# delehef/asgart

Measured on AMD Instinct MI355X. Metric: Mbp/s probe+extend (direct+RC, k=20 g=100), higher is better.
Workload: dtype u64 keys / u32 SA

## Files before the change

### asgart_amd/csrc/pipeline.hip

```cpp
#include "pipeline_dev.hpp"
#include "extend_wave_dev.hpp"
#include "extend_heavy_dev.hpp"
#include "extend_fast_dev.hpp"
#include "extend_k8_dev.hpp"

#include <algorithm>
#include <atomic>
#include <chrono>
#include <functional>
#include <string>
#include <thread>
#include <utility>

namespace asgart {

#ifdef ASGART_PROFILE_EXTEND
#define PROF_DUMP(tag)                                                                          \
    do {                                                                                       \
        fprintf(stderr, "[extend profile %s] stage=%llu batches=%llu | reg_cyc=%llu reg_probes=%llu | build=%llu "\
                "lds_probes=%llu match=%llu apply=%llu retire=%llu segs=%llu sumA=%llu sumCnt=%llu | longest: "   \
                "cyc=%llu g0=%llu lds_probes=%llu reg_probes=%llu sumA=%llu sumCnt=%llu stage=%llu match=%llu\n", \
                tag, h_ctr[16], h_ctr[17], h_ctr[18], h_ctr[19], h_ctr[20], h_ctr[21], h_ctr[22], h_ctr[23],  \
                h_ctr[24], h_ctr[25], h_ctr[26], h_ctr[27], h_ctr[28], h_ctr[29], h_ctr[30] >> 32,            \
                h_ctr[30] & 0xffffffffull, h_ctr[31] >> 32, h_ctr[31] & 0xffffffffull, h_ctr[32], h_ctr[33]); \
// ... 364 lines not shown
                    set_error("more than 2^32 probes in one call");
                    return ASGART_E_CAP;
                }
            }
            lp[(size_t)n_chunks_pass] = (uint32_t)P64;
        }
        Ppass = lp[(size_t)n_chunks_pass];
        P = Ppass * (uint32_t)n_passes;
        cx.last_P = P;
        memset(&cx.stats, 0, sizeof(cx.stats));
        cx.stats.probes_total = P;
        if (fam_out)
            for (int32_t p = 0; p < n_passes; ++p) {
                fams[p]->fam_offsets.assign(1, 0);
                fams[p]->fam_keys.clear();
                fams[p]->sds.clear();
            }
        if (want_csr) {
            status_out->assign(P, 0);
            rowoff_out->assign((size_t)P + 1, 0);
            hits_out->clear();
        }
        if (P == 0 || n_chunks == 0) return 0;
        if (want_csr && (n_shards != 1 || n_passes != 1)) {
            set_error("asgart_probe_hits is one unsharded pass");
            return ASGART_E_ARG;
        }
        own_lo = (uint32_t)((uint64_t)Ppass * (uint64_t)shard / (uint64_t)n_shards);
        own_hi = (uint32_t)((uint64_t)Ppass * (uint64_t)(shard + 1) / (uint64_t)n_shards);
        if (own_lo == own_hi) return 0;
        look_back = (uint64_t)opt.shard_lookback;
        look_ahead = opt.shard_lookahead > 0 ? (uint64_t)opt.shard_lookahead
                                                      : std::max<uint64_t>(65536, (own_hi - own_lo) / 16);
        const int64_t c0 = (int64_t)(std::upper_bound(lp.begin(), lp.end(), own_lo) - lp.begin()) - 1;
        const int64_t c1 = (int64_t)(std::upper_bound(lp.begin(), lp.end(), own_hi - 1u) - lp.begin()) - 1;
        lo_lim = lp[(size_t)c0];
        hi_lim = lp[(size_t)c1 + 1];
        K = hi_lim - lo_lim;
        for (int64_t c = 0; c < n_chunks; ++c) {
            const int64_t cl = c % n_chunks_pass, p = c / n_chunks_pass;
            h_start[c] = chunks[2 * cl];
            h_len[c] = chunks[2 * cl + 1];
            h_pbase[c] = (uint32_t)p * K + (std::min(std::max(lp[(size_t)cl], lo_lim), hi_lim) - lo_lim);
        }
        h_pbase[n_chunks] = (uint32_t)n_passes * K;
        call_sig = 1469598103934665603ull;
        {
            auto mix = [&](uint64_t v) { call_sig = (call_sig ^ v) * 1099511628211ull; };
            mix(k);
            mix(st->max_gap_size);
            mix(st->min_duplication_length);
            mix(st->max_cardinality);
            for (int64_t c = 0; c < 2 * n_chunks_pass; ++c) mix(chunks[c]);
        }
        RC_TRY(w.chunks.reserve(ch_bytes));
        d_start = w.chunks.as<uint64_t>();
        d_len = d_start + n_chunks;
        d_pbase = reinterpret_cast<uint32_t *>(d_len + n_chunks);
        HIP_TRY(hipMemcpyAsync(d_start, h_start, ch_bytes, hipMemcpyHostToDevice, s));
        t_host0 = std::chrono::steady_clock::now();
        nothing_to_do = false;
        return 0;
    }

    void set_window() {
        const uint32_t w_lo = (uint32_t)std::max<uint64_t>(lo_lim, own_lo > look_back ? own_lo - look_back : 0);
        const uint32_t w_hi = (uint32_t)std::min<uint64_t>(hi_lim, (uint64_t)own_hi + look_ahead);
        rp.init_unknown = w_lo != lo_lim ? 1u : 0u;
        rp.ch = ChunkTable{d_start, d_len, d_pbase, (int)n_chunks};
        rp.win_len = w_hi - w_lo;
        rp.win_stride = K;
        rp.g_lo = w_lo - lo_lim;
        rp.g_hi = rp.g_lo + ((uint32_t)n_passes - 1u) * K + rp.win_len;
        rp.own_off_lo = own_lo - w_lo;
        rp.own_off_hi = own_hi - w_lo;
        W = rp.g_hi - rp.g_lo;
        W_probes = (uint32_t)n_passes * rp.win_len;
        rp.k = (int)k;
        rp.step = (int)step;
        rp.G = st->max_gap_size;
        rp.tstar = (uint32_t)((st->max_gap_size + step - 1) / step);
        if (rp.tstar == 0) rp.tstar = 1;
        rp.M = st->min_duplication_length;
        rp.C = st->max_cardinality > 0xFFFFFF00ull ? 0xFFFFFF00u : (uint32_t)st->max_cardinality;
        rp.n_passes = (uint32_t)n_passes;
        rp.pass_chunks = (uint32_t)n_chunks_pass;
        rp.modes = 0;
        rp.blank = 0;
        for (int p = 0; p < 4; ++p) {
            rp.pbits[p] = nullptr;
            if (p >= n_passes) continue;
            const int mode = (sts[p].reverse ? 2 : 0) | (sts[p].complement ? 1 : 0);
            rp.modes |= (uint32_t)mode << (8 * p);
            rp.pbits[p] = opt.posbits ? idx->d_pbits[mode] : nullptr;
            if (rp.pbits[p] && idx->pbits_uses[mode] == 0) rp.blank |= 1u << p;
        }
        cx.last_rp = rp;
        cx.has_last = false;

    }

    int32_t front(bool *ambiguous) {
        const uint32_t n_blk = rp.n_tiles((uint32_t)kScanTile);
        const uint64_t seg_cap = (uint64_t)W_probes / (rp.tstar + 1) + (uint64_t)n_chunks + 64;
        RC_TRY(reserve_probe_workspace(idx, cx, W));
        RC_TRY(w.seg_list.reserve((size_t)seg_cap * 4));
        RC_TRY(w.counters.reserve(CT_COUNT * 8));
        d_ctr = w.counters.as<unsigned long long>();
        HIP_TRY(hipMemsetAsync(d_ctr, 0, CT_COUNT * 8, s));
        ix = idx->template view<SlotT>();
        p_lo = w.p_lo.as<SlotT>() - rp.g_lo;
        p_raw = w.p_raw.as<uint32_t>() - rp.g_lo;
        p_filt = w.p_filt.as<uint32_t>() - rp.g_lo;
        row_off = w.row_off.as<unsigned long long>() - rp.g_lo;
        unsigned long long *scan_desc = w.blk.as<unsigned long long>();
        uint32_t *big_list = w.big_list.as<uint32_t>();
        uint32_t *rank_list = w.rank_list.as<uint32_t>();
        seg_list = w.seg_list.as<uint32_t>();

        if (opt.test_stall_s > 0) stall_kernel<<<1, 64, 0, s>>>((unsigned long long)opt.test_stall_s * 100000000ull);
        HIP_TRY(hipEventRecord(cx.ev[EV_SEARCH], s));
        probe_count_kernel<SlotT, false><<<rp.n_tiles((uint32_t)kProbeBlock), kProbeThreads, 0, s>>>(
            ix, rp, p_lo, p_raw, p_filt, big_list, rank_list, d_ctr);
        HIP_TRY(hipEventRecord(cx.ev[EV_PROBE_COUNT], s));
        collect_pending_kernel<<<std::min<uint32_t>(rp.n_tiles((uint32_t)kCollectTile), 256u * 8u), kCollectBlock, 0, s>>>(
            rp, p_filt, big_list, rank_list, d_ctr);
        big_count_kernel<SlotT, false><<<2048, 256, 0, s>>>(ix, rp, p_lo, p_raw, p_filt, big_list, d_ctr);
        uint32_t *const ranked_top = big_list + W;
        if (ix.sap)
            rank_count_kernel<SlotT, false><<<2048, 256, 0, s>>>(ix, rp, p_lo, p_raw, p_filt, rank_list, big_list, ranked_top,
                                                                 ix.sar ? idx->ranked_fill : 0, d_ctr);
        HIP_TRY(hipEventRecord(cx.ev[EV_SEARCHED], s));
        HIP_TRY(hipMemsetAsync(scan_desc, 0, (size_t)n_blk * 16, s));
        scan_segments_kernel<<<std::min<uint32_t>(n_blk, 256u * 2u), kScanBlock, 0, s>>>(rp, p_filt, scan_desc, n_blk, row_off, seg_list, d_ctr);
        HIP_TRY(hipEventRecord(cx.ev[EV_SCANNED], s));
        HIP_TRY(hipGetLastError());
        HIP_TRY(hipMemcpyAsync(h_ctr, d_ctr, kCtrBytes, hipMemcpyDeviceToHost, s));
        RC_TRY(wd_sync(idx, cx, s, "the probe search and the scans"));
        total_hits = h_ctr[CT_TOTAL_HITS];
        n_seg = h_ctr[CT_SEG];
        if (h_ctr[CT_AMBIG]) {
            *ambiguous = true;
            return 0;
        }
        if (n_seg > seg_cap) {
            set_error("internal: segment list overflow (%llu > %llu)", (unsigned long long)n_seg,
                      (unsigned long long)seg_cap);
            return ASGART_E_CAP;
        }
        RC_TRY(w.hits.reserve((size_t)(total_hits + 64) * sizeof(SlotT)));
        hits = w.hits.as<SlotT>();
        hipStream_t sf = cx.fill_stream;
        HIP_TRY(hipEventRecord(cx.ev[EV_FILL], sf));
        fill_small_kernel<SlotT><<<rp.n_tiles(256u), 256, 0, sf>>>(ix, rp, p_lo, p_raw, p_filt, row_off, hits);
        if (h_ctr[CT_BIG])
            fill_big_kernel<SlotT><<<2048, 256, 0, sf>>>(ix, rp, p_lo, p_raw, p_filt, row_off, hits,
                                                         big_list, d_ctr);
        if constexpr (sizeof(SlotT) == 4) {
            if (h_ctr[CT_RANKED])
                fill_ranked_kernel<SlotT><<<(unsigned)std::min<uint64_t>((h_ctr[CT_RANKED] + 255) / 256, 4096), 256, 0, sf>>>(
                    ix, rp, p_lo, p_raw, p_filt, row_off, hits, ranked_top, d_ctr);
        }
        HIP_TRY(hipEventRecord(cx.ev[EV_HIT_ROWS], sf));
        HIP_TRY(hipGetLastError());

        return 0;
    }

    int32_t csr_out() {
        std::vector<uint32_t> h_filt(P);
        std::vector<SlotT> h_hits((size_t)total_hits);
        RC_TRY(wd_sync(idx, cx, s, "the hit rows"));
        HIP_TRY(hipMemcpyAsync(h_filt.data(), p_filt, (size_t)P * 4, hipMemcpyDeviceToHost, s));
        HIP_TRY(hipMemcpyAsync(rowoff_out->data(), row_off, ((size_t)P + 1) * 8,
                               hipMemcpyDeviceToHost, s));
        if (total_hits)
            HIP_TRY(hipMemcpyAsync(h_hits.data(), hits, (size_t)total_hits * sizeof(SlotT),
                                   hipMemcpyDeviceToHost, s));
        HIP_TRY(hipStreamSynchronize(s));
        for (uint32_t g = 0; g < P; ++g)
            (*status_out)[g] = h_filt[g] == kSkipN ? 1 : (h_filt[g] == kSkipCard ? 2 : 0);
        hits_out->resize((size_t)total_hits);
        for (uint64_t j = 0; j < total_hits; ++j) (*hits_out)[j] = h_hits[j];
        return 0;
    }

    int32_t place() {
        rec_cap = std::max<uint64_t>(1u << 18, w.fam_sds.cap / sizeof(SdRec));
        RC_TRY(w.ovf_list.reserve((size_t)(n_seg + 1) * 4 * kTiers));
        h_recs = nullptr;
        n_hrec = 0;
        const int force_tier = (int)opt.force_tier;
        RC_TRY(w.seg_keys.reserve((size_t)n_seg * 4 * 2));
        RC_TRY(w.seg_vals.reserve((size_t)n_seg * 4 * 2));
        uint32_t *kbuf = w.seg_keys.as<uint32_t>(), *vbuf = w.seg_vals.as<uint32_t>();
        HIP_TRY(hipMemsetAsync(d_ctr + CT_N1, 0, (size_t)(CT_COUNT - CT_N1) * 8, s));
        arms_kernel = rp.C <= (uint64_t)kHitBatch && opt.arms_kernel != 0 && (uint64_t)idx->n < (1ull << 42);
        for (int t = 1; t <= kTiers; ++t) {
            const TierShape &sh = shape(t);
            const bool usable = sh.kernel != TierKernel::none && !(arms_kernel && rp.C > (uint64_t)sh.hits);
            tier_cap[t] = usable ? (uint32_t)((uint64_t)sh.cap() * (uint64_t)(sh.widen ? opt.*sh.widen : 100) / 100u) : 0u;
        }
        tier_cap[kTiers] = 0xFFFFFFFFu;
        if (arms_kernel)
            tier_cap[3] = std::min(std::max(shape(3).cap(), tier_cap[6]), tier_cap[3]);
        else
            tier_cap[6] = (rp.G >= 0xFFF0u || rp.C >= 0xFFF0u) ? 0u : tier_cap[6] * 7 / 5;
        PlaceParams pp;
        pp.long3 = pp.long3_big = pp.dense3 = pp.dense6 = 0;
        pp.stats = opt.debug ? 1u : 0u;
        pp.barren = opt.barren ? 1u : 0u;
        pp.seg_info = nullptr;
        const bool cluster_barren = opt.barren >= 2 && rp.M > (uint64_t)k;
        split_on = opt.split >= (sizeof(SlotT) == 4 ? 1 : 2) && arms_kernel && (opt.split_len == 0 || opt.split_len >= 64);
        if (cluster_barren || split_on) {
            RC_TRY(w.seg_info.reserve((size_t)n_seg * sizeof(uint2)));
            pp.seg_info = w.seg_info.as<uint2>();
        }
        d_split = nullptr;
        if (split_on) {
            RC_TRY(w.split_buf.reserve(kSplitBytes));
            d_split = w.split_buf.as<char>();
            HIP_TRY(hipMemsetAsync(d_split, 0, 64, s));
        }
        pp.k = (uint32_t)k;
        pp.step = (uint32_t)step;
        pp.G = rp.G;
        pp.M = rp.M;
        for (int t = 1; t < kTiers; ++t) pp.cap[t - 1] = tier_cap[t];
        if (arms_kernel) {
            pp.long3 = (uint32_t)opt.long3;
            pp.long3_big = pp.long3 / 4u;
            pp.dense3 = (uint32_t)opt.dense3;
            pp.dense6 = (uint32_t)opt.dense6;
            if (force_tier == 3) {
                pp.long3 = pp.long3_big = 1;
                pp.dense3 = pp.dense6 = 0;
            }
            pp.cap[0] = (uint32_t)std::min<int64_t>(opt.cap1, shape(1).cap());
        }
        {
            int n_resident = 0;
            for (int t = 2; t < kTiers; ++t)
                n_resident += tier_enabled(t) && (shape(t).kernel == TierKernel::fast || shape(t).kernel == TierKernel::k8) ? 1 : 0;
            const bool on = tail_up.mode == 2 || (tail_up.mode == 1 && cx.n_tier_st < n_resident);
            for (int t = 1; t < kTiers; ++t) {
                const bool source = (t == 2 || t == 4 || t == 5) && shape(t).kernel == TierKernel::fast;
                const uint32_t thr = !source ? 0u : tail_up.hits > 0 ? (uint32_t)std::min<int64_t>(tail_up.hits, 0xFFFFFFFFll) : shape(t).tail_hits;
                pp.tail_hits[t - 1] = tail_hits[t] = on && tier_enabled(t) ? thr : 0u;
            }
        }
        int force_eff = force_tier;
        while (force_eff > 1 && force_eff < kTiers && !tier_enabled(force_eff)) ++force_eff;
        pp.sum1 = kTier1MaxSum;
        pp.force_tier = force_eff;
        {
            uint32_t *long_list = w.ovf_list.as<uint32_t>();
            seg_stats_lanes_kernel<<<(unsigned)std::min<uint64_t>((n_seg + 63) / 64, 256ull * 9ull * 2ull), 64, 0, s>>>(
                rp, p_filt, seg_list, d_ctr + CT_SEG, kbuf, vbuf, pp, long_list, d_ctr);
            seg_stats_kernel<<<(unsigned)std::min<uint64_t>(n_seg, 256ull * 16ull), 64, 0, s>>>(
                rp, p_filt, seg_list, d_ctr + CT_LONGSEG, long_list, kbuf, vbuf, pp, d_ctr);
        }
        HIP_TRY(hipGetLastError());
        HIP_TRY(hipStreamWaitEvent(s, cx.ev[EV_HIT_ROWS], 0));
        if (cluster_barren) {
            HIP_TRY(hipEventRecord(cx.ev[EV_BARREN], s));
            cluster_barren_kernel<SlotT, 16384><<<256 * 32, 64, 0, s>>>(rp, pp, row_off, hits, seg_list, d_ctr + CT_SEG, kbuf, 1u, 1024u,
                                                                       d_ctr + CT_CLUSTER_CUR, d_ctr);
            HIP_TRY(hipEventRecord(cx.ev[EV_BARREN_SMALL], s));
            cluster_barren_kernel<SlotT, 131072><<<256 * 9, 64, 0, s>>>(rp, pp, row_off, hits, seg_list, d_ctr + CT_SEG, kbuf, 1025u,
                                                                       16384u, d_ctr + CT_CLUSTER_CUR + 1, d_ctr);
            HIP_TRY(hipGetLastError());
            HIP_TRY(hipEventRecord(cx.ev[EV_BARREN_BIG], s));
        }
        if (split_on) {
            SplitParams sp{};
            sp.range_len = (uint32_t)opt.split_len;
            sp.warm = (uint32_t)opt.split_warm;
            sp.min_span = (uint32_t)std::min<int64_t>(opt.split_min, 0x7FFFFFFF);
            sp.max_runs = kMaxRuns - kMaxSplits;
            sp.max_cuts = kMaxCuts;
            sp.max_splits = kMaxSplits;
            {
                BlockedSeg *const h_blocked = reinterpret_cast<BlockedSeg *>(h_split + kOffBlocked);
                std::lock_guard<std::mutex> lk(idx->mu);
                for (auto b = idx->split_blocked.rbegin(); b != idx->split_blocked.rend(); ++b)
                    for (int32_t p_ = 0; p_ < n_passes && sp.n_blocked < kSplitBlockedMax; ++p_)
                        if (b->sig == call_sig && ((rp.modes >> (8 * p_)) & 0xFFu) == (uint32_t)(b->key >> 32) &&
                            (uint32_t)b->key >= lo_lim && (uint32_t)b->key < hi_lim)
                            h_blocked[sp.n_blocked++] = BlockedSeg{(uint32_t)p_ * K + ((uint32_t)b->key - lo_lim), b->range_len, b->allowed, b->warm};
            }
            sp.blocked = reinterpret_cast<const BlockedSeg *>(d_split + kOffBlocked);
            if (sp.n_blocked)
                HIP_TRY(hipMemcpyAsync(d_split + kOffBlocked, h_split + kOffBlocked, (size_t)sp.n_blocked * sizeof(BlockedSeg), hipMemcpyHostToDevice, s));
            SplitChoice *const d_choice = reinterpret_cast<SplitChoice *>(d_split + kOffChoice);
            if (!sp.range_len) {
                HIP_TRY(hipMemsetAsync(d_choice, 0, sizeof(SplitChoice), s));
                split_tally_kernel<<<grid_for(n_seg), 256, 0, s>>>(rp, d_ctr + CT_SEG, kbuf, pp.seg_info, d_choice);
                split_pick_kernel<<<1, 1, 0, s>>>(d_choice, (uint32_t)opt.split_runs);
            }
            plan_ranges_kernel<<<grid_for(n_seg), 256, 0, s>>>(rp, sp, p_filt, seg_list, d_ctr + CT_SEG, kbuf, pp.seg_info,
                                                              reinterpret_cast<unsigned long long *>(d_split),
                                                              reinterpret_cast<RangeRun *>(d_split + kOffRuns),
                                                              reinterpret_cast<uint2 *>(d_split + kOffCuts),
                                                              reinterpret_cast<SplitSeg *>(d_split + kOffSplits), d_choice);
            HIP_TRY(hipGetLastError());
            HIP_TRY(hipMemcpyAsync(h_split, d_split, kOffMeta, hipMemcpyDeviceToHost, s));
// ... 1365 lines not shown
```

### asgart_amd/csrc/pipeline_dev.hpp

```cpp
#pragma once

#include "extend_common_dev.hpp"

namespace asgart {

constexpr int kProbeBlock = 256;
constexpr int kProbeThreads = 64;
constexpr int kProbeSub = kProbeBlock / kProbeThreads;
constexpr int kMaxHalf = (kMaxKey + 1) / 2;
constexpr int kWinBytes = ((kProbeBlock + 2) * kMaxHalf + 15 + 16 + 15) / 16 * 16;

template <class SlotT, bool COUNT>
__global__ __launch_bounds__(kProbeThreads) void probe_count_kernel(IndexView<SlotT> ix, RunParams rp,
                                                                    SlotT *__restrict__ p_lo,
                                                                    uint32_t *__restrict__ p_raw,
                                                                    uint32_t *__restrict__ p_filt,
                                                                    uint32_t *__restrict__ big_list,
                                                                    uint32_t *__restrict__ rank_list,
                                                                    unsigned long long *__restrict__ ctr) {
    __shared__ __attribute__((aligned(16))) uint8_t s_text[kWinBytes];
    __shared__ uint32_t s_half[kProbeBlock + 2];
    constexpr int kPbLoads = (kProbeBlock * kMaxHalf + 127) / 128 + 2;
    __shared__ __attribute__((aligned(16))) uint32_t s_pb[kPbLoads * 4];
    __shared__ uint8_t s_surv[kProbeBlock];
    typename std::conditional<COUNT, CountBytes, NoBytes>::type cb;
    const uint32_t lane = threadIdx.x;
    const unsigned long long lt_mask = (1ull << lane) - 1ull;
    uint32_t g_end;
    const uint32_t gb = rp.tile_of(blockIdx.x, (uint32_t)kProbeBlock, g_end);
    const uint32_t g_last = min(gb + (uint32_t)kProbeBlock, g_end) - 1u;
    const int k = rp.k, H = rp.step;
    const int c0 = chunk_of_uniform(rp.ch, gb);
    const bool uniform = rp.ch.pbase[c0 + 1] > g_last && k <= kMaxKey;
    uint32_t n_rej = 0;
    auto lookup = [&](uint32_t g_, uint64_t q_, uint64_t q2_, uint64_t i_, uint64_t s_, uint64_t L_, uint32_t md_,
                      const uint64_t *lrn_) {
        const bool reverse = (md_ & 2u) != 0u, complement = (md_ & 1u) != 0u;
        uint64_t lo, hi;
        ProbeRef pr;
        pr.p = reverse ? ix.text + s_ + L_ - 1u - i_ : ix.text + s_ + i_;
        pr.dir = reverse ? -1 : 1;
        pr.comp = complement;
        const bool all_occurrences = kmer_range(ix, q_, q2_, pr, lo, hi, cb);
        const uint64_t raw = hi - lo;
        if (!COUNT) {
            p_lo[g_] = (SlotT)lo;
            p_raw[g_] = (uint32_t)raw;
        }
        cb.wr(sizeof(SlotT) + 4);
        if (raw <= (uint64_t)kSmallInterval) {
            uint32_t cnt = 0;
            const bool only_self = all_occurrences && raw == 1 && md_ == 0u;
            bool any = false;
            for (uint64_t r = lo; r < hi && !only_self; ++r) {
                cb.rd(sizeof(SlotT));
                const uint64_t x = ix.sa[r];
                cnt += keep_hit(x, i_, s_, L_, reverse) ? 1u : 0u;
                if (reverse) any |= x >= s_ + L_ - i_;
            }
            if (!reverse) any = cnt != 0u;
            if (!COUNT) p_filt[g_] = cnt > rp.C ? kSkipCard : cnt;
            cb.wr(4);
            if constexpr (!COUNT) {
                if (lrn_ && all_occurrences && !any) {
                    const uint64_t p = reverse ? s_ + L_ - i_ - (uint64_t)k : s_ + i_;
                    atomicAnd(const_cast<unsigned long long *>(reinterpret_cast<const unsigned long long *>(lrn_)) + (p >> 6),
                              ~(1ull << (p & 63u)));
                }
            }
        } else {
            if (!COUNT) p_filt[g_] = (ix.sap && all_occurrences && raw > (uint64_t)kRankMin) ? kPendingRank : kPending;
            cb.wr(4 + 4);
            cb.rd(4);
        }
    };
    auto screen = [&](uint32_t g_, uint32_t first_, bool pass_, uint32_t md_) {
        if (first_ == 4u) {
            if (!COUNT) p_filt[g_] = kSkipN;
            cb.wr(4);
            return false;
        }
        if (!pass_) {
            if (!COUNT) {
                p_raw[g_] = kRawUnknown;
                p_filt[g_] = 0u;
            }
            cb.wr(8);
            n_rej += 1;
            return false;
        }
        return true;
    };
    if (uniform) {
        const uint32_t pass0 = rp.pass_of(c0), md = rp.mode_of_pass(pass0);
        const bool reverse = (md & 2u) != 0u, complement = (md & 1u) != 0u;
        const uint64_t *const pbits = rp.pbits[pass0];
        const uint64_t s = rp.ch.start[c0], L = rp.ch.len[c0];
        const uint64_t i0 = (uint64_t)(gb - rp.ch.pbase[c0] + 1) * (uint64_t)H;
        const int n_half = kProbeBlock + 2;
        const long long b0 = (long long)(s + i0), e0 = (long long)(s + L - 1u - i0);
        const long long w_lo = reverse ? e0 - (long long)n_half * H + 1 : b0;
        const long long a_lo = w_lo & ~15ll;
        const long long w_hi = reverse ? e0 : b0 + (long long)n_half * H - 1;
        const uint32_t n_load = (uint32_t)((w_hi - a_lo) / 16 + 1);
        for (uint32_t t = lane; t < n_load; t += kProbeThreads) {
            const long long a = a_lo + 16ll * t;
            uint4 v = make_uint4(0, 0, 0, 0);
            if (a >= 0 && (uint64_t)a + 16u <= ix.n + 64u) {
                v = *reinterpret_cast<const uint4 *>(ix.text + a);
                cb.rd16();
            }
            *reinterpret_cast<uint4 *>(s_text + 16u * t) = v;
        }
        long long pb_lo = 0;
        if (pbits) {
            const long long p_first = reverse ? (long long)(s + L - i0) - k - (long long)(kProbeBlock - 1) * H
                                                 : (long long)(s + i0);
            const long long byte_lo = (p_first >> 7) * 16;
            pb_lo = byte_lo * 8;
            const long long p_last = p_first + (long long)(kProbeBlock - 1) * H;
            const uint32_t n_pb = (uint32_t)((p_last >> 7) - (p_first >> 7) + 1);
            if (lane < n_pb) {
                const long long a = byte_lo + 16ll * lane;
                uint4 v = make_uint4(~0u, ~0u, ~0u, ~0u);
                if (a >= 0 && (uint64_t)a + 16u <= ((ix.n + 63u) / 64u) * 8u + 512u) {
                    v = *reinterpret_cast<const uint4 *>(reinterpret_cast<const uint8_t *>(pbits) + a);
                    cb.rd16();
                }
                *reinterpret_cast<uint4 *>(&s_pb[4u * lane]) = v;
            }
        }
        __syncthreads();
        for (uint32_t h = lane; h < (uint32_t)n_half; h += kProbeThreads) {
            const long long p0 = reverse ? (e0 - a_lo) - (long long)h * H : (b0 - a_lo) + (long long)h * H;
            uint32_t v = 0;
            for (int j = 0; j < H; ++j) {
                uint32_t c = base_code(s_text[reverse ? p0 - j : p0 + j]);
                if (complement) c = comp_code(c);
                v = (v << 3) | c;
            }
            s_half[h] = v;
        }
        __syncthreads();
        auto key_of = [&](uint32_t t) {
            uint64_t qt = ((uint64_t)s_half[t] << (3 * H)) | (uint64_t)s_half[t + 1];
            if (k & 1) qt = (qt << 3) | (uint64_t)(s_half[t + 2] >> (3 * (H - 1)));
            return qt;
        };
        uint32_t n_surv = 0;
#pragma unroll
        for (int u = 0; u < kProbeSub; ++u) {
            const uint32_t t = lane + (uint32_t)u * kProbeThreads, g = gb + t;
            bool survivor = false;
            if (g < g_end) {
                const uint64_t q = key_of(t);
                const uint32_t first = (uint32_t)(q >> (3 * (k - 1))) & 7u;
                bool pass = true;
// ... 477 lines not shown
                if (lane == 0) scan_publish(desc, 0, kScanPre, tile_agg);
            } else {
                if (lane == 0) scan_publish(desc, tile, kScanAgg, tile_agg);
                ScanEl acc = scan_identity();
                long long hi = tile;
                for (;;) {
                    const long long t_l = hi - 64 + (long long)lane;
                    ScanEl e = scan_identity();
                    uint32_t stt = 3u;
                    if (t_l >= 0) stt = scan_peek(desc, (unsigned long long)t_l, e);
                    const unsigned long long pm = __ballot(stt == (uint32_t)kScanPre), zm = __ballot(stt == 0u);
                    const int pl = pm ? 63 - __clzll((long long)pm) : -1;
                    if (zm & lanes_above(pl)) {
                        __builtin_amdgcn_s_sleep(2);
                        continue;
                    }
                    if ((int)lane < pl || stt == 3u) e = scan_identity();
#pragma unroll
                    for (int d = 1; d < 64; d <<= 1) {
                        const ScanEl o = shfl_up_el(e, d);
                        if ((int)lane >= d) e = scan_combine(o, e);
                    }
                    acc = scan_combine(shfl_el(e, 63), acc);
                    if (pl >= 0 || hi - 64 <= 0) break;
                    hi -= 64;
                }
                excl = acc;
                if (lane == 0) scan_publish(desc, tile, kScanPre, scan_combine(excl, tile_agg));
            }
            if (lane == 0) {
                s_excl = excl;
                if (tile + 1u == n_tiles) ctr[CT_TOTAL_HITS] = excl.hits + tile_agg.hits;
            }
        }
        __syncthreads();
        ScanEl run = s_excl;
        for (uint32_t w = 0; w < wave; ++w) run = scan_combine(run, s_wave[w]);
        {
            int cn = c_first;
            uint32_t pb = pb_first;
            const uint32_t own_lo_g = g_end - rp.win_len + rp.own_off_lo, own_hi_g = g_end - rp.win_len + rp.own_off_hi;
#pragma unroll 1
            for (int r = 0; r < kScanRounds; ++r) {
                const uint32_t ga = wg0 + (uint32_t)r * 64u, g = ga + lane;
                const uint32_t fr = s_f[wave * (uint32_t)kScanWaveSpan + (uint32_t)r * 64u + lane];
                const uint32_t n_valid = ga < g_end ? min(64u, g_end - ga) : 0u;
                const bool hit = fr >= 1u && fr < kPending;
                const unsigned long long hm = __ballot(hit), qm = __ballot(fr == 0u), cardm = __ballot(fr == kSkipCard);
                unsigned long long rm = resets_of(cn, pb, ga);
                const bool syn = syn_first && r == 0;
                if (syn) rm |= 1ull;
                const uint32_t n_hit = (uint32_t)__popcll(hm), n_card = (uint32_t)__popcll(cardm);
                st_valid += n_valid;
                st_hit += n_hit;
                st_card += n_card;
                st_n += n_valid - n_hit - n_card - (uint32_t)__popcll(qm);
                const uint32_t v = hit ? fr : 0u;
                unsigned long long incl;
                if (small_counts) {
                    incl = wave_incl_scan(v);
                } else {
                    const uint32_t lo16 = wave_incl_scan(v & 0xFFFFu), hi16 = wave_incl_scan(v >> 16);
                    incl = (unsigned long long)lo16 + ((unsigned long long)hi16 << 16);
                }
                if (lane < n_valid) row_off[g] = run.hits + incl - v;
                if (lane + 1u == n_valid && g + 1u == g_end) row_off[g_end] = run.hits + incl;
                const uint32_t l_lo = own_lo_g > ga ? min(own_lo_g - ga, 64u) : 0u, l_hi = own_hi_g > ga ? min(own_hi_g - ga, 64u) : 0u;
                const unsigned long long ownm = (l_hi >= 64u ? ~0ull : (1ull << l_hi) - 1ull) & ~(l_lo >= 64u ? ~0ull : (1ull << l_lo) - 1ull);
                unsigned long long sm = 0, ambm = 0;
                if (hm & ownm) {
                    if (!rm) {
                        const uint32_t Q = __builtin_amdgcn_mbcnt_hi((uint32_t)(qm >> 32), __builtin_amdgcn_mbcnt_lo((uint32_t)qm, 0u));
                        uint32_t xp = __shfl_up(wave_incl_max_scan(hit ? Q + 1u : 0u), 1);
                        if (lane == 0u) xp = 0u;
                        const bool has_in = xp != 0u;
                        const bool unknown = !has_in && scan_unknown(run);
                        const bool has_before = has_in || (run.flags & 1u) != 0u || unknown;
                        const uint32_t quiet = has_in ? Q - (xp - 1u) : run.c + Q;
                        sm = __ballot(hit && (!has_before || quiet >= rp.tstar)) & ownm;
                        ambm = __ballot(hit && unknown && quiet < rp.tstar) & ownm;
                    } else {
                        bool start = false, amb = false;
                        scan_starts_with_resets(hit, hm, qm, rm, syn, run.c, run.flags, rp.tstar, start, amb);
                        sm = __ballot(start) & ownm;
                        ambm = __ballot(amb) & ownm;
                    }
                }
                if (ambm && lane == 0u) atomicAdd(&ctr[CT_AMBIG], (unsigned long long)__popcll(ambm));
                if (sm) {
                    uint32_t base = 0;
                    if (lane == 0) base = atomicAdd(&s_nstart, (uint32_t)__popcll(sm));
                    base = (uint32_t)__builtin_amdgcn_readfirstlane((int)base);
                    if ((sm >> lane) & 1ull) s_start[base + (uint32_t)__popcll(sm & lt_mask)] = g;
                }
                ScanEl e = round_el(hm, qm, rm, syn);
                e.hits = __shfl(incl, 63);
                run = scan_combine(run, e);
            }
        }
        __syncthreads();
        if (s_nstart > (uint32_t)(kStartCap - kScanTile)) flush_starts();
    }
    flush_starts();
    if (lane == 0) {
        atomicAdd(&sh_stat[0], st_n);
        atomicAdd(&sh_stat[1], st_card);
        atomicAdd(&sh_stat[2], st_hit);
        atomicAdd(&sh_stat[3], st_valid);
    }
    __syncthreads();
    if (tid == 0) {
        if (sh_stat[0]) atomicAdd(&ctr[CT_N_SKIPPED], sh_stat[0]);
        if (sh_stat[1]) atomicAdd(&ctr[CT_CARD_SKIPPED], sh_stat[1]);
        if (sh_stat[2]) atomicAdd(&ctr[CT_WITH_HITS], sh_stat[2]);
        if (sh_stat[3] > sh_stat[0]) atomicAdd(&ctr[CT_SEARCHED], sh_stat[3] - sh_stat[0]);
    }
}

template <class SlotT>
__global__ __launch_bounds__(256) void raw_hits_kernel(IndexView<SlotT> ix, RunParams rp, const uint32_t *__restrict__ p_filt,
                                                       const uint32_t *__restrict__ p_raw, unsigned long long *__restrict__ out) {
    unsigned long long sum = 0;
    const uint32_t n_t = rp.n_tiles(1024u);
    for (uint32_t t = blockIdx.x; t < n_t; t += gridDim.x) {
        uint32_t g_end;
        const uint32_t g0 = rp.tile_of(t, 1024u, g_end);
#pragma unroll 1
        for (int a = 0; a < 4; ++a) {
            const uint32_t g = g0 + (uint32_t)a * 256u + threadIdx.x;
            if (g >= g_end || p_filt[g] == kSkipN) continue;
            uint32_t raw = p_raw[g];
            if (raw == kRawUnknown) {
                const int c = chunk_of(rp.ch, g);
                const uint32_t md = rp.mode_of(c);
                const uint64_t cs = rp.ch.start[c], cl = rp.ch.len[c];
                const uint64_t i = (uint64_t)(g - rp.ch.pbase[c] + 1) * (uint64_t)rp.step;
                uint32_t first = 0;
                uint64_t q2 = 0, lo, hi;
                const uint64_t q = probe_key(ix.text, cs, cl, i, rp.k, (md & 2u) != 0u, (md & 1u) != 0u, &first, &q2);
                ProbeRef pr;
                pr.p = (md & 2u) ? ix.text + cs + cl - 1u - i : ix.text + cs + i;
                pr.dir = (md & 2u) ? -1 : 1;
                pr.comp = (md & 1u) != 0u;
                kmer_range(ix, q, q2, pr, lo, hi);
                raw = (uint32_t)(hi - lo);
            }
            sum += raw;
        }
    }
    for (int off = 32; off > 0; off >>= 1) sum += __shfl_down(sum, off);
    if ((threadIdx.x & 63u) == 0 && sum) atomicAdd(out, sum);
}

template <class SlotT>
__global__ __launch_bounds__(256) void fill_small_kernel(IndexView<SlotT> ix, RunParams rp,
                                                         const SlotT *__restrict__ p_lo,
                                                         const uint32_t *__restrict__ p_raw,
                                                         const uint32_t *__restrict__ p_filt,
                                                         const unsigned long long *__restrict__ row_off,
                                                         SlotT *__restrict__ hits) {
    uint32_t g_end;
    const uint32_t gb = rp.tile_of(blockIdx.x, 256u, g_end);
    const uint32_t g = gb + threadIdx.x;
    int c = chunk_of_uniform(rp.ch, gb);
    if (g >= g_end) return;
    const uint32_t f = p_filt[g];
    if (f == 0 || f >= kPending) return;
    const uint32_t raw = p_raw[g];
    if (raw > (uint32_t)kSmallInterval) return;
    while (c + 1 < rp.ch.n_chunks && g >= rp.ch.pbase[c + 1]) ++c;
    const uint64_t s = rp.ch.start[c], L = rp.ch.len[c];
    const uint64_t i = (uint64_t)(g - rp.ch.pbase[c] + 1) * (uint64_t)rp.step;
    const uint64_t lo = p_lo[g];
    unsigned long long w = row_off[g];
    for (uint32_t r = 0; r < raw; ++r) {
        const SlotT x = ix.sa[lo + r];
        if (keep_hit(x, i, s, L, (rp.mode_of(c) & 2u) != 0u)) hits[w++] = x;
    }
}

template <class SlotT>
__global__ __launch_bounds__(256) void fill_big_kernel(IndexView<SlotT> ix, RunParams rp,
                                                       const SlotT *__restrict__ p_lo,
                                                       const uint32_t *__restrict__ p_raw,
                                                       const uint32_t *__restrict__ p_filt,
                                                       const unsigned long long *__restrict__ row_off,
                                                       SlotT *__restrict__ hits,
                                                       const uint32_t *__restrict__ big_list,
                                                       const unsigned long long *__restrict__ ctr) {
    const uint32_t lane = threadIdx.x & 63u;
    const unsigned long long lt_mask = (1ull << lane) - 1ull;
    const uint64_t n_big = ctr[CT_BIG];
    const uint64_t wave = ((uint64_t)blockIdx.x * blockDim.x + threadIdx.x) >> 6;
    const uint64_t n_waves = ((uint64_t)gridDim.x * blockDim.x) >> 6;
    for (uint64_t e0 = wave * 64u; e0 < n_big; e0 += n_waves * 64u) {
        const uint32_t np = (uint32_t)min((uint64_t)64, n_big - e0);
        unsigned long long s = 0, L = 0, i = 0, lo = 0, hi = 0, w0 = 0;
        uint32_t md = 0;
        bool want = false;
        if (lane < np) {
            const uint32_t g = big_list[e0 + lane];
            const uint32_t f = p_filt[g];
            want = f != 0 && f < kPending;
            if (want) {
                const int c = chunk_of(rp.ch, g);
                md = rp.mode_of(c);
                s = rp.ch.start[c];
                L = rp.ch.len[c];
                i = (unsigned long long)(g - rp.ch.pbase[c] + 1) * (unsigned long long)rp.step;
                lo = p_lo[g];
                hi = lo + p_raw[g];
                w0 = row_off[g];
            }
        }
        unsigned long long todo = __ballot(want);
        while (todo) {
            const uint32_t p = (uint32_t)(__ffsll((long long)todo) - 1);
            todo &= todo - 1;
            const unsigned long long lo_p = lane_of(lo, p), hi_p = lane_of(hi, p), i_p = lane_of(i, p),
                                     s_p = lane_of(s, p), L_p = lane_of(L, p);
            const bool rev_p = (lane_of(md, p) & 2u) != 0u;
            unsigned long long w = lane_of(w0, p);
            for (unsigned long long base = lo_p; base < hi_p; base += 256) {
                SlotT x[4];
#pragma unroll
                for (int u = 0; u < 4; ++u) {
                    const unsigned long long r = base + 64u * u + lane;
                    x[u] = r < hi_p ? ix.sa[r] : (SlotT)0;
                }
#pragma unroll
                for (int u = 0; u < 4; ++u) {
                    const unsigned long long r = base + 64u * u + lane;
                    const bool keep = r < hi_p && keep_hit(x[u], i_p, s_p, L_p, rev_p);
                    const unsigned long long m = __ballot(keep);
                    if (keep) hits[w + __popcll(m & lt_mask)] = x[u];
                    w += __popcll(m);
                }
            }
        }
    }
}

constexpr int kRankedRounds = (kRankedCap + 1 + 63) / 64;
constexpr int kRankedWords = kRankedMaxR / 32;
__device__ inline void wave_lds_sync() {
    __builtin_amdgcn_wave_barrier();
    __asm__ volatile("s_waitcnt lgkmcnt(0)" ::: "memory");
    __builtin_amdgcn_wave_barrier();
}
template <class SlotT>
__global__ __launch_bounds__(256) void fill_ranked_kernel(IndexView<SlotT> ix, RunParams rp,
                                                          const SlotT *__restrict__ p_lo,
                                                          const uint32_t *__restrict__ p_raw,
                                                          const uint32_t *__restrict__ p_filt,
                                                          const unsigned long long *__restrict__ row_off,
                                                          SlotT *__restrict__ hits,
                                                          const uint32_t *__restrict__ ranked_top,
                                                          const unsigned long long *__restrict__ ctr) {
    static_assert(sizeof(SlotT) == 4, "32-bit slots and positions");
    __shared__ uint32_t s_bits[4][kRankedWords];
    __shared__ unsigned short s_below[4][kRankedWords];
    uint32_t *const bm = s_bits[threadIdx.x >> 6];
    unsigned short *const below = s_below[threadIdx.x >> 6];
    const uint32_t lane = threadIdx.x & 63u;
    const uint64_t n_rk = ctr[CT_RANKED];
    const uint64_t wave = ((uint64_t)blockIdx.x * blockDim.x + threadIdx.x) >> 6;
    const uint64_t n_waves = ((uint64_t)gridDim.x * blockDim.x) >> 6;
    for (uint64_t e0 = wave * 64u; e0 < n_rk; e0 += n_waves * 64u) {
        const uint32_t np = (uint32_t)min((uint64_t)64, n_rk - e0);
        unsigned long long s = 0, L = 0, i = 0, lo = 0, a0 = 0, w0 = 0;
        uint32_t md = 0, cnt = 0, R = 0;
        if (lane < np) {
            const uint32_t g = *(ranked_top - 1 - (long long)(e0 + lane));
            cnt = min(p_filt[g], (uint32_t)kRankedCap);
            R = min(p_raw[g], (uint32_t)kRankedMaxR);
            const int c = chunk_of(rp.ch, g);
            md = rp.mode_of(c);
            s = rp.ch.start[c];
            L = rp.ch.len[c];
            i = (unsigned long long)(g - rp.ch.pbase[c] + 1) * (unsigned long long)rp.step;
            lo = p_lo[g];
            a0 = R > cnt + 1u ? lo + R - cnt - 1u : lo;
            w0 = row_off[g];
        }
        SlotT xn[kRankedRounds], sn[kRankedRounds];
        auto fetch = [&](uint32_t p) {
            const unsigned long long a0_p = lane_of(a0, p), a1_p = lane_of(lo, p) + lane_of(R, p);
#pragma unroll
            for (int u = 0; u < kRankedRounds; ++u) {
                const unsigned long long r = a0_p + 64u * u + lane;
                xn[u] = r < a1_p ? ix.sap[r] : (SlotT)0;
                sn[u] = r < a1_p ? ix.sar[r] : (SlotT)0;
            }
        };
        fetch(0u);
        for (uint32_t p = 0; p < np; ++p) {
            const unsigned long long lo_p = lane_of(lo, p), a0_p = lane_of(a0, p), i_p = lane_of(i, p), s_p = lane_of(s, p),
                                     L_p = lane_of(L, p), w_p = lane_of(w0, p);
            const bool rev_p = (lane_of(md, p) & 2u) != 0u;
            const uint32_t cnt_p = lane_of(cnt, p), R_p = lane_of(R, p);
            const unsigned long long a1_p = lo_p + R_p;
            SlotT x[kRankedRounds];
            uint32_t rel[kRankedRounds];
#pragma unroll
            for (int u = 0; u < kRankedRounds; ++u) {
                const unsigned long long r = a0_p + 64u * u + lane;
                x[u] = xn[u];
                const uint32_t d = (uint32_t)sn[u] - (uint32_t)lo_p;
                rel[u] = r < a1_p && keep_hit(x[u], i_p, s_p, L_p, rev_p) && d < R_p ? d : ~0u;
            }
            if (p + 1 < np) fetch(p + 1u);
            const uint32_t nw = (R_p + 31u) >> 5;
            for (uint32_t j = lane; j < nw; j += 64u) bm[j] = 0u;
            wave_lds_sync();
#pragma unroll
            for (int u = 0; u < kRankedRounds; ++u)
                if (rel[u] != ~0u) atomicOr(&bm[rel[u] >> 5], 1u << (rel[u] & 31u));
            wave_lds_sync();
            uint32_t run = 0;
            for (uint32_t base = 0; base < nw; base += 64u) {
                const uint32_t j = base + lane;
                const uint32_t c = j < nw ? (uint32_t)__popc(bm[j]) : 0u;
                const uint32_t incl = wave_incl_scan(c);
                if (j < nw) below[j] = (unsigned short)(run + incl - c);
                run += lane_of(incl, 63u);
            }
            wave_lds_sync();
#pragma unroll
            for (int u = 0; u < kRankedRounds; ++u)
                if (rel[u] != ~0u) {
                    const uint32_t at = (uint32_t)below[rel[u] >> 5] + (uint32_t)__popc(bm[rel[u] >> 5] & ((1u << (rel[u] & 31u)) - 1u));
                    if (at < cnt_p) hits[w_p + at] = x[u];
                }
            wave_lds_sync();
        }
    }
}

constexpr int kFillAcct = 18;
__global__ __launch_bounds__(256) void fill_account_kernel(RunParams rp, const uint32_t *__restrict__ p_raw,
                                                           const uint32_t *__restrict__ p_filt,
                                                           const uint32_t *__restrict__ big_list,
                                                           const uint32_t *__restrict__ ranked_top,
                                                           unsigned long long *__restrict__ ctr) {
    unsigned long long acc[kFillAcct];
#pragma unroll
    for (int j = 0; j < kFillAcct; ++j) acc[j] = 0;
    const uint32_t n_t = rp.n_tiles(1024u);
    for (uint32_t t = blockIdx.x; t < n_t; t += gridDim.x) {
        uint32_t g_end;
        const uint32_t g0 = rp.tile_of(t, 1024u, g_end);
        for (int a = 0; a < 4; ++a) {
            const uint32_t g = g0 + (uint32_t)a * 256u + threadIdx.x;
            if (g >= g_end) continue;
            const uint32_t f = p_filt[g];
            if (f == 0 || f >= kPending) continue;
            const uint32_t raw = p_raw[g];
            if (raw > (uint32_t)kSmallInterval) continue;
            acc[0] += 1;
            acc[1] += raw;
        }
    }
    const uint64_t n_big = ctr[CT_BIG], n_big0 = ctr[CT_BIG0], n_rk = ctr[CT_RANKED];
    const uint64_t tid = (uint64_t)blockIdx.x * blockDim.x + threadIdx.x, stride = (uint64_t)gridDim.x * blockDim.x;
    for (uint64_t e = tid; e < n_big; e += stride) {
        const uint32_t g = big_list[e], f = p_filt[g];
        if (f == 0 || f >= kPending) continue;
        const unsigned long long R = p_raw[g];
        acc[2] += 1;
        acc[3] += R;
        const int cl = e >= n_big0 ? 2 : (R > (unsigned long long)kRankMin ? 1 : 0);
        acc[6 + 3 * cl] += 1;
        acc[7 + 3 * cl] += R;
        acc[8 + 3 * cl] += f;
    }
    for (uint64_t e = tid; e < n_rk; e += stride) {
        const uint32_t g = *(ranked_top - 1 - (long long)e), f = p_filt[g];
        const unsigned long long R = p_raw[g];
        acc[4] += 1;
        acc[5] += 2u * (R > (unsigned long long)f + 1u ? (unsigned long long)f + 1u : R);
        acc[15] += 1;
        acc[16] += R;
        acc[17] += f;
    }
#pragma unroll
    for (int j = 0; j < kFillAcct; ++j) {
        unsigned long long v = acc[j];
        for (int off = 32; off > 0; off >>= 1) v += __shfl_down(v, off);
        if ((threadIdx.x & 63u) == 0 && v) atomicAdd(&ctr[CT_FILL_ACCT + j], v);
    }
}

struct PlaceParams {
    uint32_t cap[kTiers - 1];
    uint32_t sum1;
    int force_tier;
    uint32_t long3;
    uint32_t long3_big;
    uint32_t dense6;
    uint32_t stats;
    uint32_t barren;
    uint2 *seg_info;
// ... 619 lines not shown
```

Baseline: 50100.

## Compact live rows per wave and fill small hit rows cooperatively

The small-row fill kernel now gives each wave a 1024-position tile. It first compacts the live rows into LDS with a ballot, then flattens all their suffix-array entries across lanes using a prefix scan and a binary search over lane offsets. Kept hits get their write rank from ballot masks, which replaces the old per-thread serial loop over each row. This targets warp divergence and the uncoalesced per-thread SA reads, at the cost of bpermute traffic and more complex rank logic.

```diff
diff --git a/asgart_amd/csrc/pipeline.hip b/asgart_amd/csrc/pipeline.hip
--- a/asgart_amd/csrc/pipeline.hip
+++ b/asgart_amd/csrc/pipeline.hip
@@ -540,7 +540,8 @@
         hits = w.hits.as<SlotT>();
         hipStream_t sf = cx.fill_stream;
         HIP_TRY(hipEventRecord(cx.ev[EV_FILL], sf));
-        fill_small_kernel<SlotT><<<rp.n_tiles(256u), 256, 0, sf>>>(ix, rp, p_lo, p_raw, p_filt, row_off, hits);
+        fill_small_kernel<SlotT><<<(rp.n_tiles((uint32_t)kFillTile) + kFillWaves - 1u) / kFillWaves, 64 * kFillWaves, 0, sf>>>(
+            ix, rp, p_lo, p_raw, p_filt, row_off, hits);
         if (h_ctr[CT_BIG])
             fill_big_kernel<SlotT><<<2048, 256, 0, sf>>>(ix, rp, p_lo, p_raw, p_filt, row_off, hits,
                                                          big_list, d_ctr);
diff --git a/asgart_amd/csrc/pipeline_dev.hpp b/asgart_amd/csrc/pipeline_dev.hpp
--- a/asgart_amd/csrc/pipeline_dev.hpp
+++ b/asgart_amd/csrc/pipeline_dev.hpp
@@ -3,6 +3,48 @@
 #include "extend_common_dev.hpp"
 
 namespace asgart {
+
+__device__ inline void wave_lds_sync() {
+    __builtin_amdgcn_wave_barrier();
+    __asm__ volatile("s_waitcnt lgkmcnt(0)" ::: "memory");
+    __builtin_amdgcn_wave_barrier();
+}
+
+struct HitRule {
+    unsigned long long thr, self;
+};
+__device__ inline HitRule hit_rule(uint64_t i, uint64_t s, uint64_t L, bool reverse) {
+    HitRule h;
+    h.thr = reverse ? s + L - i : i + s + 1u;
+    h.self = reverse ? i : ~0ull;
+    return h;
+}
+__device__ inline uint32_t lane_get(uint32_t v, uint32_t l) {
+    return (uint32_t)__builtin_amdgcn_ds_bpermute((int)(l << 2), (int)v);
+}
+__device__ inline unsigned long long lane_get(unsigned long long v, uint32_t l) {
+    return ((unsigned long long)lane_get((uint32_t)(v >> 32), l) << 32) | lane_get((uint32_t)v, l);
+}
+template <class SlotT, class F>
+__device__ inline void walk_small_rows(const SlotT *__restrict__ sa, unsigned long long lo, uint32_t raw, HitRule hr, F &&round) {
+    const uint32_t lane = threadIdx.x & 63u;
+    const uint32_t incl = wave_incl_scan(raw), pre = incl - raw;
+    const uint32_t total = lane_of(incl, 63u);
+    for (uint32_t base = 0; base < total; base += 64u) {
+        const uint32_t e = base + lane;
+        uint32_t own = 0;
+#pragma unroll
+        for (uint32_t step = 32u; step; step >>= 1)
+            if (lane_get(pre, own + step) <= e) own += step;
+        const uint32_t r = e - lane_get(pre, own);
+        const unsigned long long lo_o = lane_get(lo, own), thr_o = lane_get(hr.thr, own), self_o = lane_get(hr.self, own);
+        const bool live = e < total;
+        SlotT x = 0;
+        if (live) x = sa[lo_o + r];
+        const bool keep = live && (unsigned long long)x >= thr_o && (unsigned long long)x != self_o;
+        round(own, r, x, keep, (unsigned long long)__ballot(keep));
+    }
+}
 
 constexpr int kProbeBlock = 256;
 constexpr int kProbeThreads = 64;
@@ -786,30 +828,68 @@
     if ((threadIdx.x & 63u) == 0 && sum) atomicAdd(out, sum);
 }
 
+constexpr int kFillTile = 1024, kFillWaves = 4;
 template <class SlotT>
-__global__ __launch_bounds__(256) void fill_small_kernel(IndexView<SlotT> ix, RunParams rp,
-                                                         const SlotT *__restrict__ p_lo,
-                                                         const uint32_t *__restrict__ p_raw,
-                                                         const uint32_t *__restrict__ p_filt,
-                                                         const unsigned long long *__restrict__ row_off,
-                                                         SlotT *__restrict__ hits) {
+__global__ __launch_bounds__(64 * kFillWaves) void fill_small_kernel(IndexView<SlotT> ix, RunParams rp,
+                                                                     const SlotT *__restrict__ p_lo,
+                                                                     const uint32_t *__restrict__ p_raw,
+                                                                     const uint32_t *__restrict__ p_filt,
+                                                                     const unsigned long long *__restrict__ row_off,
+                                                                     SlotT *__restrict__ hits) {
+    __shared__ unsigned short s_rows[kFillWaves][kFillTile];
+    unsigned short *const rows = s_rows[threadIdx.x >> 6];
+    const uint32_t lane = threadIdx.x & 63u;
+    const unsigned long long lt_mask = (1ull << lane) - 1ull;
+    const uint32_t tile = uni(blockIdx.x * (uint32_t)kFillWaves + (threadIdx.x >> 6));
+    if (tile >= rp.n_tiles((uint32_t)kFillTile)) return;
     uint32_t g_end;
-    const uint32_t gb = rp.tile_of(blockIdx.x, 256u, g_end);
-    const uint32_t g = gb + threadIdx.x;
-    int c = chunk_of_uniform(rp.ch, gb);
-    if (g >= g_end) return;
-    const uint32_t f = p_filt[g];
-    if (f == 0 || f >= kPending) return;
-    const uint32_t raw = p_raw[g];
-    if (raw > (uint32_t)kSmallInterval) return;
-    while (c + 1 < rp.ch.n_chunks && g >= rp.ch.pbase[c + 1]) ++c;
-    const uint64_t s = rp.ch.start[c], L = rp.ch.len[c];
-    const uint64_t i = (uint64_t)(g - rp.ch.pbase[c] + 1) * (uint64_t)rp.step;
-    const uint64_t lo = p_lo[g];
-    unsigned long long w = row_off[g];
-    for (uint32_t r = 0; r < raw; ++r) {
-        const SlotT x = ix.sa[lo + r];
-        if (keep_hit(x, i, s, L, (rp.mode_of(c) & 2u) != 0u)) hits[w++] = x;
+    const uint32_t gb = rp.tile_of(tile, (uint32_t)kFillTile, g_end);
+    const int c0 = chunk_of_uniform(rp.ch, gb);
+    constexpr int kSub = kFillTile / 64;
+    uint32_t f[kSub];
+#pragma unroll
+    for (int u = 0; u < kSub; ++u) {
+        const uint32_t g = gb + (uint32_t)u * 64u + lane;
+        f[u] = g < g_end ? p_filt[g] : 0u;
+    }
+    uint32_t n_rows = 0;
+#pragma unroll
+    for (int u = 0; u < kSub; ++u) {
+        const bool has = f[u] != 0u && f[u] < kPending;
+        const unsigned long long m = __ballot(has);
+        if (has) rows[n_rows + (uint32_t)__popcll(m & lt_mask)] = (unsigned short)((uint32_t)u * 64u + lane);
+        n_rows += (uint32_t)__popcll(m);
+    }
+    n_rows = uni(n_rows);
+    wave_lds_sync();
+    for (uint32_t j0 = 0; j0 < n_rows; j0 += 64u) {
+        const uint32_t j = j0 + lane;
+        uint32_t raw = 0;
+        unsigned long long lo = 0, w = 0;
+        HitRule hr = {0ull, 0ull};
+        if (j < n_rows) {
+            const uint32_t g = gb + rows[j];
+            raw = p_raw[g];
+            if (raw > (uint32_t)kSmallInterval) raw = 0;
+            lo = p_lo[g];
+            w = row_off[g];
+            int c = c0;
+            while (c + 1 < rp.ch.n_chunks && g >= rp.ch.pbase[c + 1]) ++c;
+            hr = hit_rule((uint64_t)(g - rp.ch.pbase[c] + 1) * (uint64_t)rp.step, rp.ch.start[c], rp.ch.len[c],
+                          (rp.mode_of(c) & 2u) != 0u);
+        }
+        unsigned long long km_prev = 0;
+        walk_small_rows(ix.sa, lo, raw, hr,
+                        [&](uint32_t own, uint32_t r, SlotT x, bool keep, unsigned long long km) {
+                            const unsigned long long w_o = lane_get(w, own);
+                            if (keep) {
+                                const uint32_t here = min(r, lane);
+                                uint32_t rank = (uint32_t)__popcll(km & lt_mask & ~((1ull << (lane - here)) - 1ull));
+                                if (r > here) rank += (uint32_t)__popcll(km_prev >> (64u - (r - here)));
+                                hits[w_o + rank] = x;
+                            }
+                            km_prev = km;
+                        });
     }
 }
 
@@ -877,11 +957,6 @@
 
 constexpr int kRankedRounds = (kRankedCap + 1 + 63) / 64;
 constexpr int kRankedWords = kRankedMaxR / 32;
-__device__ inline void wave_lds_sync() {
-    __builtin_amdgcn_wave_barrier();
-    __asm__ volatile("s_waitcnt lgkmcnt(0)" ::: "memory");
-    __builtin_amdgcn_wave_barrier();
-}
 template <class SlotT>
 __global__ __launch_bounds__(256) void fill_ranked_kernel(IndexView<SlotT> ix, RunParams rp,
                                                           const SlotT *__restrict__ p_lo,
```

Measured after the change: 51060, median of 6. 1.02x the previous value.
